# ooowedyn/InkLayer

Hardware: AMD Instinct MI355X
Metric: sketches/sec end-to-end (GroundingDINO+SAM) at 1024x1024 (higher is better)
Workload: dtype f16 (MFMA, f32 accumulate; f32 residual/norm/softmax; split-f16 = fp32-grade operands for patch-embed, neck, mask decoder); 1 GPU; full GroundingDINO Swin-T + SAM ViT-H pipeline, batch=8 per GPU, 1024x1024 synthetic sketches, 16 boxes/sketch, random-init weights; global_batch=8, parallelism=image-parallel x1

## Files before the change

### inklayer_amd/csrc/fusion_fold.hip

```cpp
#include "common.h"
#include "../../include/inklayer_hip.h"

namespace {

constexpr int FD = 256;
constexpr int FH = 4;
constexpr int FHD = 256;
constexpr int FJ = 16;

__device__ __forceinline__ float wave_reduce16(float (&v)[16], int lane) {
  float a8[8], a4[4], a2[2];
#pragma unroll
  for (int i = 0; i < 8; ++i) {
    const bool up = lane & 32;
    const float keep = up ? v[8 + i] : v[i], give = up ? v[i] : v[8 + i];
    a8[i] = keep + __shfl_xor(give, 32, 64);
  }
#pragma unroll
  for (int i = 0; i < 4; ++i) {
    const bool up = lane & 16;
    const float keep = up ? a8[4 + i] : a8[i], give = up ? a8[i] : a8[4 + i];
    a4[i] = keep + __shfl_xor(give, 16, 64);
  }
#pragma unroll
  for (int i = 0; i < 2; ++i) {
    const bool up = lane & 8;
    const float keep = up ? a4[2 + i] : a4[i], give = up ? a4[i] : a4[2 + i];
    a2[i] = keep + __shfl_xor(give, 8, 64);
  }
  const bool up = lane & 4;
  const float keep = up ? a2[1] : a2[0], give = up ? a2[0] : a2[1];
  float r = keep + __shfl_xor(give, 4, 64);
  r += __shfl_xor(r, 2, 64);
  r += __shfl_xor(r, 1, 64);
  return r;
}

__global__ __launch_bounds__(256) void fuse_prep_kernel(const float* __restrict__ K, const float* __restrict__ VL,
                                                        int64_t ldk, const f16* __restrict__ Wq,
                                                        const float* __restrict__ bq, const f16* __restrict__ Wo,
                                                        int T, float scale, float* __restrict__ U,
                                                        float* __restrict__ c, float* __restrict__ Z) {
  __shared__ float kk[FHD], vv[FHD], red[4];
  const int j = blockIdx.x, b = blockIdx.y, h = j >> 2, t = j & 3, i = threadIdx.x;
  const bool live = t < T;
  kk[i] = live ? K[((int64_t)b * T + t) * ldk + h * FHD + i] : 0.f;
  vv[i] = live ? VL[((int64_t)b * T + t) * ldk + h * FHD + i] : 0.f;
  __syncthreads();
  float u = 0.f, z = 0.f;
  for (int d = 0; d < FHD; ++d) u = fmaf((float)Wq[(int64_t)(h * FHD + d) * FD + i], kk[d], u);
  const f16* wo = Wo + (int64_t)i * (FH * FHD) + h * FHD;
  for (int d = 0; d < FHD; d += 8) {
    const f16x8 w8 = *(const f16x8*)(wo + d);
#pragma unroll
    for (int e = 0; e < 8; ++e) z = fmaf((float)w8[e], vv[d + e], z);
  }
  U[((int64_t)b * FJ + j) * FD + i] = u * scale;
  Z[((int64_t)b * FJ + j) * FD + i] = z;
  float cb = wave_sum(bq[h * FHD + i] * kk[i]);
  if ((i & 63) == 0) red[i >> 6] = cb;
  __syncthreads();
  if (i == 0) c[b * FJ + j] = live ? (red[0] + red[1] + red[2] + red[3]) * scale : -1.0e30f;
}

constexpr int TPW = 16;
__global__ __launch_bounds__(256) void fuse_ln_scores_kernel(float* __restrict__ x, int S, const float* __restrict__ g,
                                                             const float* __restrict__ be, float eps,
                                                             const float* __restrict__ U, const float* __restrict__ c,
                                                             float* __restrict__ scores) {
  const int b = blockIdx.y, lane = threadIdx.x & 63, wave = threadIdx.x >> 6;
  f32x4 u[FJ];
#pragma unroll
  for (int j = 0; j < FJ; ++j) u[j] = *(const f32x4*)(U + ((int64_t)b * FJ + j) * FD + lane * 4);
  const f32x4 gv = *(const f32x4*)(g + lane * 4), bv = *(const f32x4*)(be + lane * 4);
  const float cj = c[b * FJ + (lane >> 2)];
  const int s0 = (blockIdx.x * 4 + wave) * TPW, s1 = min(S, s0 + TPW);
  if (s0 >= S) return;
  f32x4 nxt = *(const f32x4*)(x + ((int64_t)b * S + s0) * FD + lane * 4);
  for (int s = s0; s < s1; ++s) {
    float* row = x + ((int64_t)b * S + s) * FD + lane * 4;
    f32x4 v = nxt;
    if (s + 1 < s1) nxt = *(const f32x4*)(row + FD);
    const float mean = wave_sum((v[0] + v[1]) + (v[2] + v[3])) * (1.0f / FD);
    const f32x4 d = v - mean;
    const float var = wave_sum((d[0] * d[0] + d[1] * d[1]) + (d[2] * d[2] + d[3] * d[3])) * (1.0f / FD);
    const float rstd = 1.0f / sqrtf(var + eps);
    v = d * rstd * gv + bv;
    *(f32x4*)row = v;
    float part[16];
#pragma unroll
    for (int j = 0; j < FJ; ++j) part[j] = (v[0] * u[j][0] + v[1] * u[j][1]) + (v[2] * u[j][2] + v[3] * u[j][3]);
    const float sc = wave_reduce16(part, lane) + cj;
    if ((lane & 3) == 0) scores[((int64_t)b * S + s) * FJ + (lane >> 2)] = sc;
  }
}

__global__ __launch_bounds__(256) void fuse_apply_kernel(float* __restrict__ x, int S, int tok_per_wg,
                                                         const float* __restrict__ scores,
                                                         const float* __restrict__ stats, const float* __restrict__ Z,
                                                         const float* __restrict__ gamma, const float* __restrict__ bo,
                                                         float* __restrict__ partial, const float* __restrict__ pos,
                                                         f16* __restrict__ out16_pos, f16* __restrict__ out16) {
  __shared__ __attribute__((aligned(16))) float red[FJ * FD];
  const int b = blockIdx.y, chunk = blockIdx.x, nchunk = gridDim.x, lane = threadIdx.x & 63, wave = threadIdx.x >> 6;
  f32x4 z[FJ];
#pragma unroll
  for (int q = 0; q < FJ; ++q) z[q] = *(const f32x4*)(Z + ((int64_t)b * FJ + q) * FD + lane * 4);
  const f32x4 gv = *(const f32x4*)(gamma + lane * 4), ov = *(const f32x4*)(bo + lane * 4);
  const int j = lane >> 2;
  const float cmax = stats[((int64_t)b * FJ + j) * 2];
  f32x4 acc[FJ];
#pragma unroll
  for (int q = 0; q < FJ; ++q) acc[q] = (f32x4){0.f, 0.f, 0.f, 0.f};
  const int s_lo = chunk * tok_per_wg, s_hi = min(S, s_lo + tok_per_wg);
  float sc_n = 0.f;
  f32x4 v_n = {0.f, 0.f, 0.f, 0.f};
  if (s_lo + wave < s_hi) {
    sc_n = scores[((int64_t)b * S + s_lo + wave) * FJ + j];
    v_n = *(const f32x4*)(x + ((int64_t)b * S + s_lo + wave) * FD + lane * 4);
  }
  for (int s = s_lo + wave; s < s_hi; s += 4) {
    const float sc = sc_n;
    const f32x4 v = v_n;
    if (s + 4 < s_hi) {
      sc_n = scores[((int64_t)b * S + s + 4) * FJ + j];
      v_n = *(const f32x4*)(x + ((int64_t)b * S + s + 4) * FD + lane * 4);
    }
    float mx = fmaxf(sc, __shfl_xor(sc, 4, 64));
    mx = fmaxf(mx, __shfl_xor(mx, 8, 64));
    const float e = expf(sc - mx);
    float sum = e + __shfl_xor(e, 4, 64);
    sum += __shfl_xor(sum, 8, 64);
    const float pv = e / sum, wl = expf(sc - cmax);
    float* row = x + ((int64_t)b * S + s) * FD + lane * 4;
    f32x4 o = ov;
#pragma unroll
    for (int q = 0; q < FJ; ++q) {
      const float p = __builtin_bit_cast(float, __builtin_amdgcn_readlane(__builtin_bit_cast(int, pv), 4 * q));
      const float w = __builtin_bit_cast(float, __builtin_amdgcn_readlane(__builtin_bit_cast(int, wl), 4 * q));
      o += p * z[q];
      acc[q] += w * v;
    }
    const f32x4 nv = v + gv * o;
    *(f32x4*)row = nv;
    if (out16) *(f16x4*)(out16 + ((int64_t)b * S + s) * FD + lane * 4) = (f16x4){(f16)nv[0], (f16)nv[1], (f16)nv[2], (f16)nv[3]};
    if (out16_pos) {
      const f32x4 pv4 = nv + *(const f32x4*)(pos + (int64_t)s * FD + lane * 4);
      *(f16x4*)(out16_pos + ((int64_t)b * S + s) * FD + lane * 4) = (f16x4){(f16)pv4[0], (f16)pv4[1], (f16)pv4[2], (f16)pv4[3]};
    }
  }
  for (int wv = 0; wv < 4; ++wv) {
    if (wave == wv) {
#pragma unroll
      for (int q = 0; q < FJ; ++q) {
        f32x4* dst = (f32x4*)(red + q * FD + lane * 4);
        *dst = wv == 0 ? acc[q] : *dst + acc[q];
      }
    }
    __syncthreads();
  }
  float* out = partial + ((int64_t)b * nchunk + chunk) * FJ * FD;
  for (int i = threadIdx.x; i < FJ * FD / 4; i += 256) ((f32x4*)out)[i] = ((const f32x4*)red)[i];
}

__global__ __launch_bounds__(1024) void fuse_text_kernel(const float* __restrict__ partial, int nchunk,
                                                         const float* __restrict__ stats, const f16* __restrict__ Wvv,
                                                         const float* __restrict__ bvv, int T, f16* __restrict__ out_l) {
  __shared__ __attribute__((aligned(16))) float part[4][FD];
  __shared__ __attribute__((aligned(16))) float m[FD];
  const int j = blockIdx.x, b = blockIdx.y, h = j >> 2, t = j & 3, i = threadIdx.x & 255, grp = threadIdx.x >> 8;
  if (t >= T) return;
  float s0 = 0.f, s1 = 0.f;
  int c = grp;
  for (; c + 4 < nchunk; c += 8) {
    s0 += partial[(((int64_t)b * nchunk + c) * FJ + j) * FD + i];
    s1 += partial[(((int64_t)b * nchunk + c + 4) * FJ + j) * FD + i];
  }
  if (c < nchunk) s0 += partial[(((int64_t)b * nchunk + c) * FJ + j) * FD + i];
  part[grp][i] = s0 + s1;
  __syncthreads();
  if (grp == 0) m[i] = ((part[0][i] + part[1][i]) + (part[2][i] + part[3][i])) / stats[((int64_t)b * FJ + j) * 2 + 1];
  __syncthreads();
  if (grp != 0) return;
  const f16* wr = Wvv + (int64_t)(h * FHD + i) * FD;
  float o = bvv[h * FHD + i];
  for (int d = 0; d < FD; d += 8) {
    const f16x8 w8 = *(const f16x8*)(wr + d);
#pragma unroll
    for (int e = 0; e < 8; ++e) o = fmaf((float)w8[e], m[d + e], o);
  }
  out_l[((int64_t)b * T + t) * (FH * FHD) + h * FHD + i] = (f16)o;
}

}

extern "C" int ink_fusion_fold_workspace(int32_t B, int32_t S, int64_t* out_floats) {
  INK_CHECK_ARG(out_floats && B > 0 && S > 0);
  const int64_t nchunk = (S + 127) / 128;
  *out_floats = 2 * (int64_t)B * FJ * FD + (int64_t)B * FJ + (int64_t)B * S * FJ + (int64_t)B * FJ * 2 +
                (int64_t)B * 64 * FJ * 2 + (int64_t)B * nchunk * FJ * FD;
  return INK_OK;
}

extern "C" int ink_biattn_colstats(const float* scores, int32_t B, int32_t S, int32_t HT, float* part_ws, float* stats,
                                   void* stream);

extern "C" int ink_fusion_fold(float* v_f32, int32_t B, int32_t S, const float* lnv_g, const float* lnv_b, float eps,
                               const float* text_k_f32, const float* text_vl_f32, int64_t ld_text, int32_t T,
                               const void* Wq_f16, const float* bq, const void* Wvv_f16, const float* bvv,
                               const void* Wo_f16, const float* bo, const float* gamma_v, float scale, float* ws,
                               void* out_l_f16, const float* pos, void* out16_pos, void* out16, void* stream) {
  INK_CHECK_ARG(v_f32 && lnv_g && lnv_b && text_k_f32 && text_vl_f32 && Wq_f16 && bq && Wvv_f16 && bvv && Wo_f16 && bo &&
                gamma_v && ws && out_l_f16);
  INK_CHECK_ARG(B > 0 && S > 0 && S <= 64 * 512 && T >= 1 && T <= 4 && ld_text >= FH * FHD);
  INK_CHECK_ARG(!out16_pos || pos);
  hipStream_t s = (hipStream_t)stream;
  const int nchunk = (S + 127) / 128;
  float* U = ws;
  float* Z = U + (int64_t)B * FJ * FD;
  float* c = Z + (int64_t)B * FJ * FD;
  float* scores = c + (int64_t)B * FJ;
  float* stats = scores + (int64_t)B * S * FJ;
  float* cpart = stats + (int64_t)B * FJ * 2;
  float* partial = cpart + (int64_t)B * 64 * FJ * 2;
  hipLaunchKernelGGL(fuse_prep_kernel, dim3(FJ, B), dim3(256), 0, s, text_k_f32, text_vl_f32, ld_text,
                     (const f16*)Wq_f16, bq, (const f16*)Wo_f16, T, scale, U, c, Z);
  hipLaunchKernelGGL(fuse_ln_scores_kernel, dim3((S + 4 * TPW - 1) / (4 * TPW), B), dim3(256), 0, s, v_f32, S, lnv_g,
                     lnv_b, eps, (const float*)U, (const float*)c, scores);
  if (ink_biattn_colstats(scores, B, S, FJ, cpart, stats, stream) != INK_OK) return INK_ERR_LAUNCH;
  hipLaunchKernelGGL(fuse_apply_kernel, dim3(nchunk, B), dim3(256), 0, s, v_f32, S, 128, (const float*)scores,
                     (const float*)stats, (const float*)Z, gamma_v, bo, partial, pos, (f16*)out16_pos, (f16*)out16);
  hipLaunchKernelGGL(fuse_text_kernel, dim3(FJ, B), dim3(1024), 0, s, (const float*)partial, nchunk, (const float*)stats,
                     (const f16*)Wvv_f16, bvv, T, (f16*)out_l_f16);
  return ink_launch_status();
}
```

Baseline: 118.4 sketches/s.

## Fuse LN, scores, column softmax and apply into one MFMA token kernel

The separate layernorm+scores kernel, the column-statistics pass and the apply kernel are merged into a single per-chunk kernel. It computes scores and the output and accumulator products with fp32 MFMA 16x16x4 instead of shuffle reductions, using an online (flash-style) column softmax with per-chunk max/sum stats. The text kernel then rescales the per-chunk partials. This removes the scores round-trip through global memory, one x read/write and two launches, at the cost of LDS staging, wave-level syncs and a changed fp32 summation order.

```diff
diff --git a/inklayer_amd/csrc/fusion_fold.hip b/inklayer_amd/csrc/fusion_fold.hip
--- a/inklayer_amd/csrc/fusion_fold.hip
+++ b/inklayer_amd/csrc/fusion_fold.hip
@@ -8,32 +8,14 @@
 constexpr int FHD = 256;
 constexpr int FJ = 16;
 
-__device__ __forceinline__ float wave_reduce16(float (&v)[16], int lane) {
-  float a8[8], a4[4], a2[2];
-#pragma unroll
-  for (int i = 0; i < 8; ++i) {
-    const bool up = lane & 32;
-    const float keep = up ? v[8 + i] : v[i], give = up ? v[i] : v[8 + i];
-    a8[i] = keep + __shfl_xor(give, 32, 64);
-  }
-#pragma unroll
-  for (int i = 0; i < 4; ++i) {
-    const bool up = lane & 16;
-    const float keep = up ? a8[4 + i] : a8[i], give = up ? a8[i] : a8[4 + i];
-    a4[i] = keep + __shfl_xor(give, 16, 64);
-  }
-#pragma unroll
-  for (int i = 0; i < 2; ++i) {
-    const bool up = lane & 8;
-    const float keep = up ? a4[2 + i] : a4[i], give = up ? a4[i] : a4[2 + i];
-    a2[i] = keep + __shfl_xor(give, 8, 64);
-  }
-  const bool up = lane & 4;
-  const float keep = up ? a2[1] : a2[0], give = up ? a2[0] : a2[1];
-  float r = keep + __shfl_xor(give, 4, 64);
-  r += __shfl_xor(r, 2, 64);
-  r += __shfl_xor(r, 1, 64);
-  return r;
+constexpr int TOK = 128;
+constexpr int RLD = FD + 4;
+constexpr int TLD = 20;
+
+__device__ __forceinline__ int fuse_ch(int i, int g) { return (i >> 1) * 32 + g * 8 + (i & 1) * 4; }
+
+__device__ __forceinline__ f32x4 mfma4(float a, float b, f32x4 c) {
+  return __builtin_amdgcn_mfma_f32_16x16x4f32(a, b, c, 0, 0, 0);
 }
 
 __global__ __launch_bounds__(256) void fuse_prep_kernel(const float* __restrict__ K, const float* __restrict__ VL,
@@ -55,131 +37,255 @@
 #pragma unroll
     for (int e = 0; e < 8; ++e) z = fmaf((float)w8[e], vv[d + e], z);
   }
-  U[((int64_t)b * FJ + j) * FD + i] = u * scale;
-  Z[((int64_t)b * FJ + j) * FD + i] = z;
+  const int tile = (i >> 5) * 2 + ((i >> 2) & 1), g = (i >> 3) & 3, e = i & 3;
+  U[(int64_t)b * FJ * FD + ((tile * 64 + g * 16 + j) * 4 + e)] = u * scale;
+  Z[(int64_t)b * FJ * FD + ((tile * 64 + (j >> 2) * 16 + g * 4 + e) * 4 + (j & 3))] = z;
   float cb = wave_sum(bq[h * FHD + i] * kk[i]);
   if ((i & 63) == 0) red[i >> 6] = cb;
   __syncthreads();
   if (i == 0) c[b * FJ + j] = live ? (red[0] + red[1] + red[2] + red[3]) * scale : -1.0e30f;
 }
 
-constexpr int TPW = 16;
-__global__ __launch_bounds__(256) void fuse_ln_scores_kernel(float* __restrict__ x, int S, const float* __restrict__ g,
-                                                             const float* __restrict__ be, float eps,
-                                                             const float* __restrict__ U, const float* __restrict__ c,
-                                                             float* __restrict__ scores) {
-  const int b = blockIdx.y, lane = threadIdx.x & 63, wave = threadIdx.x >> 6;
-  f32x4 u[FJ];
-#pragma unroll
-  for (int j = 0; j < FJ; ++j) u[j] = *(const f32x4*)(U + ((int64_t)b * FJ + j) * FD + lane * 4);
-  const f32x4 gv = *(const f32x4*)(g + lane * 4), bv = *(const f32x4*)(be + lane * 4);
-  const float cj = c[b * FJ + (lane >> 2)];
-  const int s0 = (blockIdx.x * 4 + wave) * TPW, s1 = min(S, s0 + TPW);
-  if (s0 >= S) return;
-  f32x4 nxt = *(const f32x4*)(x + ((int64_t)b * S + s0) * FD + lane * 4);
-  for (int s = s0; s < s1; ++s) {
-    float* row = x + ((int64_t)b * S + s) * FD + lane * 4;
-    f32x4 v = nxt;
-    if (s + 1 < s1) nxt = *(const f32x4*)(row + FD);
-    const float mean = wave_sum((v[0] + v[1]) + (v[2] + v[3])) * (1.0f / FD);
-    const f32x4 d = v - mean;
-    const float var = wave_sum((d[0] * d[0] + d[1] * d[1]) + (d[2] * d[2] + d[3] * d[3])) * (1.0f / FD);
-    const float rstd = 1.0f / sqrtf(var + eps);
-    v = d * rstd * gv + bv;
-    *(f32x4*)row = v;
-    float part[16];
-#pragma unroll
-    for (int j = 0; j < FJ; ++j) part[j] = (v[0] * u[j][0] + v[1] * u[j][1]) + (v[2] * u[j][2] + v[3] * u[j][3]);
-    const float sc = wave_reduce16(part, lane) + cj;
-    if ((lane & 3) == 0) scores[((int64_t)b * S + s) * FJ + (lane >> 2)] = sc;
-  }
-}
-
-__global__ __launch_bounds__(256) void fuse_apply_kernel(float* __restrict__ x, int S, int tok_per_wg,
-                                                         const float* __restrict__ scores,
-                                                         const float* __restrict__ stats, const float* __restrict__ Z,
-                                                         const float* __restrict__ gamma, const float* __restrict__ bo,
-                                                         float* __restrict__ partial, const float* __restrict__ pos,
+__device__ __forceinline__ void wave_lds_sync() {
+  __builtin_amdgcn_fence(__ATOMIC_RELEASE, "wavefront");
+  __builtin_amdgcn_wave_barrier();
+  __builtin_amdgcn_fence(__ATOMIC_ACQUIRE, "wavefront");
+}
+
+__global__ __launch_bounds__(256) void fuse_token_kernel(float* __restrict__ x, int S, const float* __restrict__ g,
+                                                         const float* __restrict__ be, float eps,
+                                                         const float* __restrict__ U, const float* __restrict__ c,
+                                                         const float* __restrict__ Z, const float* __restrict__ gamma,
+                                                         const float* __restrict__ bo, float* __restrict__ partial,
+                                                         float* __restrict__ cstat, const float* __restrict__ pos,
                                                          f16* __restrict__ out16_pos, f16* __restrict__ out16) {
-  __shared__ __attribute__((aligned(16))) float red[FJ * FD];
-  const int b = blockIdx.y, chunk = blockIdx.x, nchunk = gridDim.x, lane = threadIdx.x & 63, wave = threadIdx.x >> 6;
-  f32x4 z[FJ];
-#pragma unroll
-  for (int q = 0; q < FJ; ++q) z[q] = *(const f32x4*)(Z + ((int64_t)b * FJ + q) * FD + lane * 4);
-  const f32x4 gv = *(const f32x4*)(gamma + lane * 4), ov = *(const f32x4*)(bo + lane * 4);
-  const int j = lane >> 2;
-  const float cmax = stats[((int64_t)b * FJ + j) * 2];
-  f32x4 acc[FJ];
-#pragma unroll
-  for (int q = 0; q < FJ; ++q) acc[q] = (f32x4){0.f, 0.f, 0.f, 0.f};
-  const int s_lo = chunk * tok_per_wg, s_hi = min(S, s_lo + tok_per_wg);
-  float sc_n = 0.f;
-  f32x4 v_n = {0.f, 0.f, 0.f, 0.f};
-  if (s_lo + wave < s_hi) {
-    sc_n = scores[((int64_t)b * S + s_lo + wave) * FJ + j];
-    v_n = *(const f32x4*)(x + ((int64_t)b * S + s_lo + wave) * FD + lane * 4);
-  }
-  for (int s = s_lo + wave; s < s_hi; s += 4) {
-    const float sc = sc_n;
-    const f32x4 v = v_n;
-    if (s + 4 < s_hi) {
-      sc_n = scores[((int64_t)b * S + s + 4) * FJ + j];
-      v_n = *(const f32x4*)(x + ((int64_t)b * S + s + 4) * FD + lane * 4);
-    }
-    float mx = fmaxf(sc, __shfl_xor(sc, 4, 64));
-    mx = fmaxf(mx, __shfl_xor(mx, 8, 64));
-    const float e = expf(sc - mx);
-    float sum = e + __shfl_xor(e, 4, 64);
-    sum += __shfl_xor(sum, 8, 64);
-    const float pv = e / sum, wl = expf(sc - cmax);
-    float* row = x + ((int64_t)b * S + s) * FD + lane * 4;
-    f32x4 o = ov;
-#pragma unroll
-    for (int q = 0; q < FJ; ++q) {
-      const float p = __builtin_bit_cast(float, __builtin_amdgcn_readlane(__builtin_bit_cast(int, pv), 4 * q));
-      const float w = __builtin_bit_cast(float, __builtin_amdgcn_readlane(__builtin_bit_cast(int, wl), 4 * q));
-      o += p * z[q];
-      acc[q] += w * v;
-    }
-    const f32x4 nv = v + gv * o;
-    *(f32x4*)row = nv;
-    if (out16) *(f16x4*)(out16 + ((int64_t)b * S + s) * FD + lane * 4) = (f16x4){(f16)nv[0], (f16)nv[1], (f16)nv[2], (f16)nv[3]};
-    if (out16_pos) {
-      const f32x4 pv4 = nv + *(const f32x4*)(pos + (int64_t)s * FD + lane * 4);
-      *(f16x4*)(out16_pos + ((int64_t)b * S + s) * FD + lane * 4) = (f16x4){(f16)pv4[0], (f16)pv4[1], (f16)pv4[2], (f16)pv4[3]};
-    }
-  }
+  __shared__ __attribute__((aligned(16))) float sUZ[2 * FJ * FD];
+  __shared__ __attribute__((aligned(16))) float sv[4 * FD];
+  __shared__ __attribute__((aligned(16))) float sT[4][2][16 * TLD];
+  __shared__ __attribute__((aligned(16))) float sW[4][16 * TLD];
+  __shared__ __attribute__((aligned(16))) float sWM[4][FJ];
+  __shared__ __attribute__((aligned(16))) float sWL[4][FJ];
+  static_assert(FJ * RLD <= 2 * FJ * FD, "the combine buffer reuses the U | Z staging area");
+  const int b = blockIdx.y, chunk = blockIdx.x, nchunk = gridDim.x;
+  const int lane = threadIdx.x & 63, wave = threadIdx.x >> 6, tok = lane & 15, kg = lane >> 4;
+  for (int i = threadIdx.x; i < FJ * FD / 4; i += 256) {
+    ((f32x4*)sUZ)[i] = ((const f32x4*)(U + (int64_t)b * FJ * FD))[i];
+    ((f32x4*)sUZ)[FJ * FD / 4 + i] = ((const f32x4*)(Z + (int64_t)b * FJ * FD))[i];
+  }
+  sv[threadIdx.x] = g[threadIdx.x];
+  sv[FD + threadIdx.x] = be[threadIdx.x];
+  sv[2 * FD + threadIdx.x] = gamma[threadIdx.x];
+  sv[3 * FD + threadIdx.x] = bo[threadIdx.x];
+  __syncthreads();
+  const float* sU = sUZ;
+  const float* sZ = sUZ + FJ * FD;
+  float* myW = sW[wave];
+  const f32x4 cj = *(const f32x4*)(c + b * FJ + kg * 4);
+  const int s_lo = chunk * TOK, s_hi = min(S, s_lo + TOK);
+  f32x4 acc[16];
+#pragma unroll
+  for (int n = 0; n < 16; ++n) acc[n] = (f32x4){0.f, 0.f, 0.f, 0.f};
+  f32x4 Mr = {-3.0e38f, -3.0e38f, -3.0e38f, -3.0e38f}, lsum = {0.f, 0.f, 0.f, 0.f};
+  float Mrj = -3.0e38f;
+#pragma unroll 1
+  for (int p = 0; p < TOK / 64; ++p) {
+    const int t0 = s_lo + (p * 4 + wave) * 16;
+    if (t0 >= s_hi) break;
+    const int s = t0 + tok;
+    const bool valid = s < s_hi;
+    const int64_t r = (int64_t)b * S + (valid ? s : t0);
+    const float* row = x + r * FD;
+    f32x4 xr[16];
+#pragma unroll
+    for (int i = 0; i < 16; ++i) xr[i] = *(const f32x4*)(row + fuse_ch(i, kg));
+    float ps[16];
+#pragma unroll
+    for (int i = 0; i < 16; ++i) ps[i] = (xr[i][0] + xr[i][1]) + (xr[i][2] + xr[i][3]);
+#pragma unroll
+    for (int w = 8; w > 0; w >>= 1)
+#pragma unroll
+      for (int i = 0; i < w; ++i) ps[i] += ps[i + w];
+    float sum = ps[0];
+    sum += __shfl_xor(sum, 16, 64);
+    sum += __shfl_xor(sum, 32, 64);
+    const float mean = sum * (1.0f / FD);
+#pragma unroll
+    for (int i = 0; i < 16; ++i) {
+      xr[i] = xr[i] - mean;
+      ps[i] = (xr[i][0] * xr[i][0] + xr[i][1] * xr[i][1]) + (xr[i][2] * xr[i][2] + xr[i][3] * xr[i][3]);
+    }
+#pragma unroll
+    for (int w = 8; w > 0; w >>= 1)
+#pragma unroll
+      for (int i = 0; i < w; ++i) ps[i] += ps[i + w];
+    float var = ps[0];
+    var += __shfl_xor(var, 16, 64);
+    var += __shfl_xor(var, 32, 64);
+    const float rstd = 1.0f / sqrtf(var * (1.0f / FD) + eps);
+    f32x4 sa = {0.f, 0.f, 0.f, 0.f}, sb = {0.f, 0.f, 0.f, 0.f};
+#pragma unroll
+    for (int i = 0; i < 16; ++i) {
+      const int ch = fuse_ch(i, kg);
+      xr[i] = xr[i] * rstd * *(const f32x4*)(sv + ch) + *(const f32x4*)(sv + FD + ch);
+      const f32x4 uu = *(const f32x4*)(sU + (i * 64 + lane) * 4);
+#pragma unroll
+      for (int e = 0; e < 4; ++e) {
+        if (i & 1) sb = mfma4(uu[e], xr[i][e], sb);
+        else sa = mfma4(uu[e], xr[i][e], sa);
+      }
+    }
+    const f32x4 sc = (sa + sb) + cj;
+    const float mx = fmaxf(fmaxf(sc[0], sc[1]), fmaxf(sc[2], sc[3]));
+    f32x4 pv;
+#pragma unroll
+    for (int q = 0; q < 4; ++q) pv[q] = expf(sc[q] - mx);
+    const float den = (pv[0] + pv[1]) + (pv[2] + pv[3]);
+#pragma unroll
+    for (int q = 0; q < 4; ++q) pv[q] = pv[q] / den;
+    f32x4 mp;
+#pragma unroll
+    for (int q = 0; q < 4; ++q) mp[q] = valid ? sc[q] : -3.0e38f;
+#pragma unroll
+    for (int o = 1; o < 16; o <<= 1)
+#pragma unroll
+      for (int q = 0; q < 4; ++q) mp[q] = fmaxf(mp[q], __shfl_xor(mp[q], o, 64));
+    const float mps = (tok & 2) ? ((tok & 1) ? mp[3] : mp[2]) : ((tok & 1) ? mp[1] : mp[0]);
+    const float mpj = __shfl(mps, (tok >> 2) * 16 + tok, 64);
+    f32x4 w;
+#pragma unroll
+    for (int q = 0; q < 4; ++q) {
+      const float mn = fmaxf(Mr[q], mp[q]);
+      w[q] = valid ? expf(sc[q] - mn) : 0.f;
+      lsum[q] = lsum[q] * expf(Mr[q] - mn) + w[q];
+      Mr[q] = mn;
+    }
+    const float mnj = fmaxf(Mrj, mpj), fj = expf(Mrj - mnj);
+    Mrj = mnj;
+#pragma unroll
+    for (int n = 0; n < 16; ++n) acc[n] = acc[n] * fj;
+    wave_lds_sync();
+    *(f32x4*)(myW + tok * TLD + kg * 4) = w;
+    wave_lds_sync();
+    float wb[4];
+#pragma unroll
+    for (int q = 0; q < 4; ++q) wb[q] = myW[(4 * kg + q) * TLD + tok];
+    float* xo = x + r * FD;
+#pragma unroll
+    for (int n2 = 0; n2 < 8; ++n2) {
+      f32x4 nv[2];
+#pragma unroll
+      for (int hh = 0; hh < 2; ++hh) {
+        const int n = 2 * n2 + hh, ch = fuse_ch(n, kg);
+        const f32x4 zz = *(const f32x4*)(sZ + (n * 64 + lane) * 4);
+        f32x4 o = *(const f32x4*)(sv + 3 * FD + ch);
+#pragma unroll
+        for (int q = 0; q < 4; ++q) o = mfma4(zz[q], pv[q], o);
+        nv[hh] = xr[n] + *(const f32x4*)(sv + 2 * FD + ch) * o;
+        float* T = sT[wave][hh];
+        *(f32x4*)(T + tok * TLD + kg * 4) = xr[n];
+      }
+      wave_lds_sync();
+#pragma unroll
+      for (int hh = 0; hh < 2; ++hh) {
+        const int n = 2 * n2 + hh;
+        const float* T = sT[wave][hh];
+#pragma unroll
+        for (int q = 0; q < 4; ++q) acc[n] = mfma4(T[(4 * kg + q) * TLD + tok], wb[q], acc[n]);
+      }
+      wave_lds_sync();
+      if (valid) {
+        const int ch = fuse_ch(2 * n2, kg);
+        *(f32x4*)(xo + ch) = nv[0];
+        *(f32x4*)(xo + ch + 4) = nv[1];
+        if (out16)
+          *(f16x8*)(out16 + r * FD + ch) = (f16x8){(f16)nv[0][0], (f16)nv[0][1], (f16)nv[0][2], (f16)nv[0][3],
+                                                   (f16)nv[1][0], (f16)nv[1][1], (f16)nv[1][2], (f16)nv[1][3]};
+        if (out16_pos) {
+          const f32x4 q0 = nv[0] + *(const f32x4*)(pos + (int64_t)s * FD + ch);
+          const f32x4 q1 = nv[1] + *(const f32x4*)(pos + (int64_t)s * FD + ch + 4);
+          *(f16x8*)(out16_pos + r * FD + ch) = (f16x8){(f16)q0[0], (f16)q0[1], (f16)q0[2], (f16)q0[3],
+                                                       (f16)q1[0], (f16)q1[1], (f16)q1[2], (f16)q1[3]};
+        }
+      }
+    }
+  }
+#pragma unroll
+  for (int o = 1; o < 16; o <<= 1)
+#pragma unroll
+    for (int q = 0; q < 4; ++q) lsum[q] += __shfl_xor(lsum[q], o, 64);
+  if (tok == 0) {
+    *(f32x4*)(&sWM[wave][kg * 4]) = Mr;
+    *(f32x4*)(&sWL[wave][kg * 4]) = lsum;
+  }
+  __syncthreads();
+  const float Mc = fmaxf(fmaxf(sWM[0][tok], sWM[1][tok]), fmaxf(sWM[2][tok], sWM[3][tok]));
+  const float fw = expf(Mrj - Mc);
+  float* red = sUZ;
   for (int wv = 0; wv < 4; ++wv) {
     if (wave == wv) {
 #pragma unroll
-      for (int q = 0; q < FJ; ++q) {
-        f32x4* dst = (f32x4*)(red + q * FD + lane * 4);
-        *dst = wv == 0 ? acc[q] : *dst + acc[q];
+      for (int n = 0; n < 16; ++n) {
+        f32x4* dst = (f32x4*)(red + tok * RLD + fuse_ch(n, kg));
+        const f32x4 a = acc[n] * fw;
+        *dst = wv == 0 ? a : *dst + a;
       }
     }
     __syncthreads();
   }
   float* out = partial + ((int64_t)b * nchunk + chunk) * FJ * FD;
-  for (int i = threadIdx.x; i < FJ * FD / 4; i += 256) ((f32x4*)out)[i] = ((const f32x4*)red)[i];
+  for (int i = threadIdx.x; i < FJ * FD / 4; i += 256) ((f32x4*)out)[i] = *(const f32x4*)(red + (i >> 6) * RLD + (i & 63) * 4);
+  if (threadIdx.x < FJ) {
+    const int j = threadIdx.x;
+    const float M = fmaxf(fmaxf(sWM[0][j], sWM[1][j]), fmaxf(sWM[2][j], sWM[3][j]));
+    const float L = (sWL[0][j] * expf(sWM[0][j] - M) + sWL[1][j] * expf(sWM[1][j] - M)) +
+                    (sWL[2][j] * expf(sWM[2][j] - M) + sWL[3][j] * expf(sWM[3][j] - M));
+    float* cs = cstat + (((int64_t)b * nchunk + chunk) * FJ + j) * 2;
+    cs[0] = M;
+    cs[1] = L;
+  }
 }
 
 __global__ __launch_bounds__(1024) void fuse_text_kernel(const float* __restrict__ partial, int nchunk,
-                                                         const float* __restrict__ stats, const f16* __restrict__ Wvv,
+                                                         const float* __restrict__ cstat, const f16* __restrict__ Wvv,
                                                          const float* __restrict__ bvv, int T, f16* __restrict__ out_l) {
   __shared__ __attribute__((aligned(16))) float part[4][FD];
   __shared__ __attribute__((aligned(16))) float m[FD];
+  __shared__ float sf[256], sl[64], sred[2];
   const int j = blockIdx.x, b = blockIdx.y, h = j >> 2, t = j & 3, i = threadIdx.x & 255, grp = threadIdx.x >> 8;
+  const int tid = threadIdx.x;
   if (t >= T) return;
+  const float* cs = cstat + ((int64_t)b * nchunk * FJ + j) * 2;
+  if (tid < 64) {
+    float mx = -3.0e38f;
+    for (int c = tid; c < nchunk; c += 64) mx = fmaxf(mx, cs[(int64_t)c * FJ * 2]);
+    mx = wave_max(mx);
+    if (tid == 0) sred[0] = mx;
+  }
+  __syncthreads();
+  if (tid < 256) sf[tid] = tid < nchunk ? expf(cs[(int64_t)tid * FJ * 2] - sred[0]) : 0.f;
+  __syncthreads();
+  if (tid < 64) {
+    float l[4];
+#pragma unroll
+    for (int q = 0; q < 4; ++q) l[q] = tid * 4 + q < nchunk ? cs[(int64_t)(tid * 4 + q) * FJ * 2 + 1] * sf[tid * 4 + q] : 0.f;
+    sl[tid] = (l[0] + l[1]) + (l[2] + l[3]);
+  }
   float s0 = 0.f, s1 = 0.f;
   int c = grp;
   for (; c + 4 < nchunk; c += 8) {
-    s0 += partial[(((int64_t)b * nchunk + c) * FJ + j) * FD + i];
-    s1 += partial[(((int64_t)b * nchunk + c + 4) * FJ + j) * FD + i];
-  }
-  if (c < nchunk) s0 += partial[(((int64_t)b * nchunk + c) * FJ + j) * FD + i];
+    s0 += partial[(((int64_t)b * nchunk + c) * FJ + j) * FD + i] * sf[c];
+    s1 += partial[(((int64_t)b * nchunk + c + 4) * FJ + j) * FD + i] * sf[c + 4];
+  }
+  if (c < nchunk) s0 += partial[(((int64_t)b * nchunk + c) * FJ + j) * FD + i] * sf[c];
   part[grp][i] = s0 + s1;
   __syncthreads();
-  if (grp == 0) m[i] = ((part[0][i] + part[1][i]) + (part[2][i] + part[3][i])) / stats[((int64_t)b * FJ + j) * 2 + 1];
+  if (tid == 0) {
+    float L = 0.f;
+    for (int q = 0; q < (nchunk + 3) / 4; ++q) L += sl[q];
+    sred[1] = L;
+  }
+  __syncthreads();
+  if (grp == 0) m[i] = ((part[0][i] + part[1][i]) + (part[2][i] + part[3][i])) / sred[1];
   __syncthreads();
   if (grp != 0) return;
   const f16* wr = Wvv + (int64_t)(h * FHD + i) * FD;
@@ -197,13 +303,9 @@
 extern "C" int ink_fusion_fold_workspace(int32_t B, int32_t S, int64_t* out_floats) {
   INK_CHECK_ARG(out_floats && B > 0 && S > 0);
   const int64_t nchunk = (S + 127) / 128;
-  *out_floats = 2 * (int64_t)B * FJ * FD + (int64_t)B * FJ + (int64_t)B * S * FJ + (int64_t)B * FJ * 2 +
-                (int64_t)B * 64 * FJ * 2 + (int64_t)B * nchunk * FJ * FD;
+  *out_floats = 2 * (int64_t)B * FJ * FD + (int64_t)B * FJ + (int64_t)B * nchunk * FJ * 2 + (int64_t)B * nchunk * FJ * FD;
   return INK_OK;
 }
-
-extern "C" int ink_biattn_colstats(const float* scores, int32_t B, int32_t S, int32_t HT, float* part_ws, float* stats,
-                                   void* stream);
 
 extern "C" int ink_fusion_fold(float* v_f32, int32_t B, int32_t S, const float* lnv_g, const float* lnv_b, float eps,
                                const float* text_k_f32, const float* text_vl_f32, int64_t ld_text, int32_t T,
@@ -219,18 +321,13 @@
   float* U = ws;
   float* Z = U + (int64_t)B * FJ * FD;
   float* c = Z + (int64_t)B * FJ * FD;
-  float* scores = c + (int64_t)B * FJ;
-  float* stats = scores + (int64_t)B * S * FJ;
-  float* cpart = stats + (int64_t)B * FJ * 2;
-  float* partial = cpart + (int64_t)B * 64 * FJ * 2;
+  float* cstat = c + (int64_t)B * FJ;
+  float* partial = cstat + (int64_t)B * nchunk * FJ * 2;
   hipLaunchKernelGGL(fuse_prep_kernel, dim3(FJ, B), dim3(256), 0, s, text_k_f32, text_vl_f32, ld_text,
                      (const f16*)Wq_f16, bq, (const f16*)Wo_f16, T, scale, U, c, Z);
-  hipLaunchKernelGGL(fuse_ln_scores_kernel, dim3((S + 4 * TPW - 1) / (4 * TPW), B), dim3(256), 0, s, v_f32, S, lnv_g,
-                     lnv_b, eps, (const float*)U, (const float*)c, scores);
-  if (ink_biattn_colstats(scores, B, S, FJ, cpart, stats, stream) != INK_OK) return INK_ERR_LAUNCH;
-  hipLaunchKernelGGL(fuse_apply_kernel, dim3(nchunk, B), dim3(256), 0, s, v_f32, S, 128, (const float*)scores,
-                     (const float*)stats, (const float*)Z, gamma_v, bo, partial, pos, (f16*)out16_pos, (f16*)out16);
-  hipLaunchKernelGGL(fuse_text_kernel, dim3(FJ, B), dim3(1024), 0, s, (const float*)partial, nchunk, (const float*)stats,
+  hipLaunchKernelGGL(fuse_token_kernel, dim3(nchunk, B), dim3(256), 0, s, v_f32, S, lnv_g, lnv_b, eps, (const float*)U,
+                     (const float*)c, (const float*)Z, gamma_v, bo, partial, cstat, pos, (f16*)out16_pos, (f16*)out16);
+  hipLaunchKernelGGL(fuse_text_kernel, dim3(FJ, B), dim3(1024), 0, s, (const float*)partial, nchunk, (const float*)cstat,
                      (const f16*)Wvv_f16, bvv, T, (f16*)out_l_f16);
   return ink_launch_status();
 }
```

Result: no change. 119.4 sketches/s, median of 6 (+0.8%).
